# ostafen/smart

Measured on AMD Instinct MI355X. Metric: GB/s text scanned per GPU (bit-exact occ count), m=32 on 1 GiB rand128, higher is better.
Workload: dtype u8; 1 GPU; HOR m=32, 1.00 GiB rand128 per GPU; algorithm=hor, m=32, sigma=128, text_bytes_per_gpu=1073741824, patterns=2668, corpus=counter-based splitmix64 rand-sigma, seed 0x5EED0001, generated on device, ranks=1

## Files before the change

### smart_amd/csrc/api.cpp

```cpp
#include "../../include/smartgpu.h"

#include <hip/hip_runtime.h>
#include <rccl/rccl.h>

#include <dlfcn.h>

#include <algorithm>
#include <atomic>
#include <chrono>
#include <condition_variable>
#include <functional>
#include <mutex>
#include <thread>
#include <cstdarg>
#include <cstdio>
#include <cstring>
#include <string>
#include <vector>

#include "kernels.hpp"
#include "multi.hpp"
#include "pedit.hpp"
#include "peditl.hpp"
#include "tedit.hpp"
// ... 210 lines not shown
    if (e != hipSuccess) { set_error("text_alphabet failed: %s", hipGetErrorString(e)); return false; }
    t->rate = with_rate ? sg::text_repeat_rate(hist) : -1.0;
    if (!sg::four_symbol_codes(t->alphabet, &t->four_shift, &t->four_symtab)) t->four_shift = 7;
    t->one_bit = 0xFF;
    {
        uint32_t syms[3], ns = 0;
        for (uint32_t c = 0; c < 256 && ns < 3; ++c)
            if (t->alphabet[c >> 5] >> (c & 31) & 1u) syms[ns++] = c;
        if (ns == 1) syms[ns++] = syms[0];
        if (ns == 2) {
            uint32_t bit = 0;
            while (bit < 7 && ((syms[0] ^ syms[1]) >> bit & 1u) == 0) ++bit;
            const uint32_t s0 = (syms[0] >> bit & 1u) ? syms[1] : syms[0], s1 = (syms[0] >> bit & 1u) ? syms[0] : syms[1];
            t->one_bit = bit | (s0 << 8) | (s1 << 16);
        }
    }
    const uint32_t words[3] = {t->four_shift, t->four_symtab, t->one_bit};
    if (hipMemcpyAsync(t->base, words, 12, hipMemcpyHostToDevice, d->stream) != hipSuccess ||
        hipMemsetAsync(dev, 0, 32, d->stream) != hipSuccess ||
        hipStreamSynchronize(d->stream) != hipSuccess) {
        set_error("text_alphabet: writing the codes failed");
        return false;
    }
    return true;
}

bool text_no_alphabet(smartgpu_text* t, DeviceCtx* d)
{
    t->four_shift = 7;
    t->four_symtab = 0;
    t->one_bit = 0xFF;
    t->rate = -1.0;
    for (uint32_t& wv : t->alphabet) wv = 0xFFFFFFFFu;
    const uint32_t words[3] = {7u, 0u, 0xFFu};
    if (hipMemcpyAsync(t->base, words, 12, hipMemcpyHostToDevice, d->stream) != hipSuccess || hipStreamSynchronize(d->stream) != hipSuccess) {
        set_error("text upload: writing the codes failed");
        return false;
    }
    return true;
}

std::atomic<long long> g_text_sampling{64ll << 20};

void text_sample(smartgpu_text* t, DeviceCtx* d)
{
    const long long least = g_text_sampling.load(std::memory_order_relaxed);
    if (least < 0 || t->n < static_cast<uint64_t>(least) || !sg::g_sample_build) return;
    uint32_t* s = nullptr;
    if (hipMalloc(reinterpret_cast<void**>(&s), sg::sample_alloc_dwords(t->n) * 4) != hipSuccess) {
        (void)hipGetLastError();
        return;
    }
    if (sg::g_sample_build(t->data(), t->n, s, d->num_cus, d->stream) != hipSuccess || hipStreamSynchronize(d->stream) != hipSuccess) {
        (void)hipGetLastError();
        (void)hipFree(s);
        return;
    }
    t->sample = s;
}

int check_pattern(int algo, const uint8_t* P, uint32_t m, bool length_first = false)
{
    if (algo < 0 || algo >= SMARTGPU_NUM_ALGOS) { set_error("unknown algorithm id %d", algo); return SMARTGPU_ERR_ARG; }
    const bool na = m < sg::min_pattern(algo);
    if ((!na || length_first) && (!P || m < 1 || m > SMARTGPU_XSIZE)) { set_error("pattern length %u outside [1,%d]", m, SMARTGPU_XSIZE); return SMARTGPU_ERR_ARG; }
    if (na) { set_error("%s: not applicable for m < %u", sg::kAlgoNames[algo], sg::min_pattern(algo)); return SMARTGPU_NA; }
    return SMARTGPU_OK;
}

int check_search_args(int algo, const uint8_t* P, uint32_t m, const smartgpu_text* text,
                      uint64_t off, uint64_t n)
{
    const int rc = check_pattern(algo, P, m);
    if (rc != SMARTGPU_OK) return rc;
    if (!text) { set_error("text handle is NULL"); return SMARTGPU_ERR_ARG; }
    if (off > text->n || n > text->n - off) { set_error("range [%llu,+%llu) outside the text (%llu bytes)", (unsigned long long)off, (unsigned long long)n, (unsigned long long)text->n); return SMARTGPU_ERR_ARG; }
    return SMARTGPU_OK;
}

sg::ScanArgs make_args(const sg::PlanWords& pw, uint32_t m, const uint8_t* blob, unsigned long long* count, const smartgpu_text* text,
                       uint64_t off, uint64_t n)
{
    const uint64_t s_end = (n >= m) ? off + n - m + 1 : off;
    return sg::ScanArgs{text->data(), off, s_end, m, pw.halo,  0, pw.prefer_packed, pw.sparse, pw.so_off, blob, count};
}

struct QueuedScan { int algo; sg::ScanArgs a; sg::TextCodes codes; uint8_t tail[sg::kTailRow]; uint8_t head[sg::kSampleRow]; const uint32_t* sample; };
bool same_key(const sg::ScanArgs& x, const sg::ScanArgs& a) { return x.text == a.text && x.s_begin == a.s_begin && x.s_end == a.s_end && x.m == a.m && x.halo == a.halo; }
struct QueuedKey {
    sg::ScanArgs key;
    uint32_t n = 0;
    uint32_t streaming = 0;
    int64_t opened_ns = 0;
    bool fast = false;
    QueuedScan scans[sg::kLongMax];
    bool holds(const sg::ScanArgs& a) const { return same_key(key, a); }
    void take(const QueuedKey& o)
    {
        key = o.key;
        n = o.n;
        streaming = o.streaming;
        opened_ns = o.opened_ns;
        fast = o.fast;
        std::memcpy(static_cast<void*>(scans), static_cast<const void*>(o.scans), o.n * sizeof(QueuedScan));
    }
};
static_assert(std::is_trivially_copyable<QueuedScan>::value, "QueuedKey::take copies entries as bytes");
static_assert(SMARTGPU_XSIZE - 1 - sg::kGramCap + sg::kTailRow <= sg::kPatternBytes, "a long pass reads whole rows from a blob's pattern slot");
struct LaunchQueue {
    std::mutex mu;
    static constexpr uint32_t kKeys = 8;
    uint32_t nkeys = 0;
    QueuedKey keys[kKeys];
    void drop(uint32_t at) { for (--nkeys; at < nkeys; ++at) keys[at].take(keys[at + 1]); }
    uint32_t nfull = 0, full_next = 0;
    sg::ScanArgs full[kKeys];
    bool was_full(const sg::ScanArgs& a) const
    {
        for (uint32_t i = 0; i < nfull; ++i)
            if (same_key(full[i], a)) return true;
        return false;
    }
    void note_full(const sg::ScanArgs& a)
    {
        if (was_full(a)) return;
        if (nfull < kKeys) { full[nfull++] = a; return; }
        full[full_next] = a;
        full_next = (full_next + 1) % kKeys;
    }
    bool off = false;
    uint64_t launches = 0, passes = 0;
    uint64_t riders = 0;
    uint64_t sampled = 0;
};
LaunchQueue g_queue[kMaxDevices];
std::atomic<long long> g_coalesce_long{64ll << 20};
constexpr int kCoalesceNarrow = 8;
std::atomic<int> g_coalesce{sg::kPassMax};
std::atomic<int> g_coalesce_sample{1};
std::atomic<int> g_sample_grid{0};
bool pass_sampled(const uint32_t* sample, uint32_t m)
{
    return sample && m >= sg::kSampleMinM && sg::g_hor_sample && g_coalesce_sample.load(std::memory_order_relaxed) != 0;
}

int64_t host_ns()
{
    return std::chrono::duration_cast<std::chrono::nanoseconds>(std::chrono::steady_clock::now().time_since_epoch()).count();
}
constexpr int64_t kFastLeastNs = 10000;
int64_t pass_estimate_ns(uint64_t range, bool sampled)
{
    const uint64_t bytes = sampled ? range / (sg::kSampleStride / sg::kSampleGram) : range;
    return static_cast<int64_t>(bytes / 4400u);
}

hipError_t send_key(const DeviceCtx* d, LaunchQueue& q, QueuedKey& k)
{
    hipError_t e = k.n ? hipSetDevice(d->device) : hipSuccess;
    if (e != hipSuccess) {
        k.n = 0;
        k.streaming = 0;
        return e;
    }
    if (k.n == 1) {
        e = sg::launch_scan(k.scans[0].algo, k.scans[0].a, d->num_cus, d->stream, k.scans[0].codes);
    } else if (k.n > 1) {
        sg::MultiArgs ma;
        ma.text = k.key.text;
        ma.s_begin = k.key.s_begin;
        ma.s_end = k.key.s_end;
        ma.m = k.key.m;
        ma.halo = k.key.halo & 0xFFu;
        ma.np = k.n;
        const uint32_t* sample = k.scans[0].sample;
        if (pass_sampled(sample, k.key.m)) {
            const bool by_value = k.n <= sg::kSampleWidth;
            ma.stride = sg::kSampleRow;
            ma.width = by_value ? sg::kSampleWidth : sg::kSampleLongWidth;
            ma.reserved = by_value ? sg::kMultiByValue : sg::kMultiLong;
            for (uint32_t j = 0; j < k.n; ++j) {
                if (by_value) sg::sample_set(ma, j, k.scans[j].a.blob, k.scans[j].a.count, k.scans[j].head);
                else sg::multi_set_long(ma, j, k.scans[j].a.blob, k.scans[j].a.count);
            }
            e = sg::g_hor_sample(ma, sample, d->num_cus, g_sample_grid.load(std::memory_order_relaxed), d->stream);
            if (e == hipSuccess) ++q.sampled;
        } else {
            ma.stride = sg::tail_stride(k.key.m);
            if (k.n <= sg::pass_width(k.key.m)) {
                ma.width = sg::pass_width(k.key.m);
                ma.reserved = sg::kMultiByValue;
                for (uint32_t j = 0; j < k.n; ++j) sg::multi_set(ma, j, k.scans[j].a.blob, k.scans[j].a.count, k.scans[j].tail);
            } else {
                ma.width = sg::long_width(k.key.m);
                ma.reserved = sg::kMultiLong;
                for (uint32_t j = 0; j < k.n; ++j) sg::multi_set_long(ma, j, k.scans[j].a.blob, k.scans[j].a.count);
            }
            e = sg::g_hor_multi(ma, d->num_cus, d->stream);
        }
    }
    if (k.n && e == hipSuccess) ++q.passes;
    k.n = 0;
    k.streaming = 0;
    return e;
}

hipError_t flush_queue(const DeviceCtx* d)
{
    LaunchQueue& q = g_queue[d->device];
    std::lock_guard<std::mutex> lock(q.mu);
    hipError_t err = hipSuccess;
    for (uint32_t i = 0; i < q.nkeys; ++i) {
        const hipError_t e = send_key(d, q, q.keys[i]);
        if (e != hipSuccess && err == hipSuccess) err = e;
    }
    q.nkeys = 0;
    q.nfull = q.full_next = 0;
    return err;
}

void flush_all_queues()
{
    int current = -1;
    for (int i = 0; i < kMaxDevices; ++i) {
        if (!g_dev[i].ready) continue;
        {
            std::lock_guard<std::mutex> lock(g_queue[i].mu);
            if (g_queue[i].nkeys == 0) continue;
        }
        if (current < 0 && hipGetDevice(&current) != hipSuccess) return;
        if (hipSetDevice(i) == hipSuccess) (void)flush_queue(&g_dev[i]);
    }
    if (current >= 0) (void)hipSetDevice(current);
}

DeviceCtx* device_ctx_flushed(int device)
{
    DeviceCtx* d = device_ctx(device);
    if (!d) return nullptr;
    const hipError_t e = flush_queue(d);
    if (e != hipSuccess) { set_error("a queued launch failed: %s", hipGetErrorString(e)); return nullptr; }
    return d;
}

hipError_t queue_launch(const DeviceCtx* d, int algo, const sg::PlanWords& words, const sg::ScanArgs& a, const sg::TextCodes& codes,
                        double text_rate, const uint8_t (&tail)[sg::kTailRow], const uint8_t (&head)[sg::kSampleRow], const uint32_t* sample,
                        bool timed, bool* queued)
{
    *queued = false;
    if (a.s_end <= a.s_begin) return hipSuccess;
    const bool rider = !words.sparse;
    if (rider && (a.m < 8 || !sg::text_rate_streams(text_rate))) return hipSuccess;
    const sg::Route r = sg::route(algo, a.m, words, codes);
    if (r.to != sg::Launcher::hor || r.arg != 0) return hipSuccess;
    LaunchQueue& q = g_queue[d->device];
    std::lock_guard<std::mutex> lock(q.mu);
    if (!rider) ++q.launches;
    const int G = g_coalesce.load(std::memory_order_relaxed);
    if (timed || G < 2 || q.off || !sg::g_hor_multi) {
        if (!rider) ++q.passes;
        return hipSuccess;
    }
    hipError_t err = hipSuccess;
    uint32_t at = 0;
    while (at < q.nkeys && !q.keys[at].holds(a)) ++at;
    if (at == q.nkeys) {
        if (rider) return hipSuccess;
        if (q.nkeys == LaunchQueue::kKeys) {
            err = send_key(d, q, q.keys[0]);
            q.drop(0);
        }
        at = q.nkeys++;
        q.keys[at].key = a;
        q.keys[at].n = 0;
        q.keys[at].streaming = 0;
        q.keys[at].fast = false;
        q.keys[at].opened_ns = host_ns();
    }
    QueuedKey& k = q.keys[at];
    QueuedScan& qs = k.scans[k.n++];
    qs.algo = algo;
    qs.a = a;
    qs.codes = codes;
    std::memcpy(qs.tail, tail, sg::kTailRow);
    std::memcpy(qs.head, head, sg::kSampleRow);
    qs.sample = sample;
    if (rider) ++q.riders; else ++k.streaming;
    const bool sampled = pass_sampled(sample, a.m);
    const uint32_t room = sampled ? sg::kSampleWidth : sg::pass_width(a.m);
    const uint32_t long_room = sampled ? sg::kSampleLongWidth : sg::long_width(a.m);
    const uint32_t width = static_cast<uint32_t>(G) < room ? static_cast<uint32_t>(G) : room;
    const long long least = g_coalesce_long.load(std::memory_order_relaxed);
    const bool may_gather = G == sg::kPassMax && least >= 0 && a.s_end - a.s_begin >= static_cast<uint64_t>(least);
    const bool full = k.streaming >= width || k.n >= room;
    if (may_gather && full && !k.fast && k.n < long_room && !q.was_full(a)) {
        const int64_t waited = host_ns() - k.opened_ns;
        const int64_t pass_ns = pass_estimate_ns(a.s_end - a.s_begin, sampled);
        k.fast = pass_ns >= kFastLeastNs && waited >= 0 && waited / k.n * (long_room - k.n) < pass_ns;
    }
    const bool gather_on = may_gather && (k.fast || q.was_full(a));
    if (gather_on ? k.n >= long_room : full) {
        q.note_full(k.key);
        const hipError_t e = send_key(d, q, k);
        if (e != hipSuccess && err == hipSuccess) err = e;
        q.drop(at);
    }
    *queued = true;
// ... 2481 lines not shown
```

### smart_amd/csrc/k_hors.hip

```cpp
#include "dev_common.hpp"
#include "launch_common.hpp"
#include "sample.hpp"

namespace sg {

__global__ __launch_bounds__(256) void text_sample_build(const uint8_t* text, uint64_t count, uint64_t alloc, uint32_t* sample)
{
    const uint64_t step = (uint64_t)gridDim.x * 256;
    for (uint64_t k = (uint64_t)blockIdx.x * 256 + threadIdx.x; k < alloc; k += step)
        sample[k] = k < count ? __builtin_nontemporal_load(reinterpret_cast<const uint32_t*>(text + k * kSampleStride)) : 0u;
}

static hipError_t launch_sample_build(const uint8_t* text, uint64_t n, uint32_t* sample, int num_cus, hipStream_t stream)
{
    const uint64_t alloc = sample_alloc_dwords(n), want = (alloc + 255) / 256;
    const uint32_t grid = (uint32_t)std::max<uint64_t>(1, std::min<uint64_t>(want, (uint64_t)num_cus * 16));
    hipLaunchKernelGGL(text_sample_build, dim3(grid), dim3(256), 0, stream, text, sample_count(n), alloc, sample);
    return hipGetLastError();
}

constexpr int kHorsInFlight = 4;
constexpr uint32_t kHorsLaneVerify = 64;
constexpr uint32_t kHorsGramsPerThread = (kSampleLongWidth * kSampleStride + kSampleThreads - 1) / kSampleThreads;

__device__ __forceinline__ const uint8_t* hors_global(unsigned long long v)
{
    typedef const __attribute__((address_space(1))) uint8_t* global_u8;
    return (const uint8_t*)reinterpret_cast<global_u8>(v);
}
__device__ __forceinline__ unsigned long long hors_area64(const MultiArgs& a, uint32_t at)
{
    return *reinterpret_cast<const unsigned long long*>(a.area + at);
}
__device__ __forceinline__ unsigned long long hors_lane(unsigned long long v, int src)
{
    const uint32_t lo = __builtin_amdgcn_readlane((uint32_t)v, src), hi = __builtin_amdgcn_readlane((uint32_t)(v >> 32), src);
    return ((unsigned long long)hi << 32) | lo;
}
__device__ __forceinline__ uint32_t hors_wave_verify(bool has, const uint8_t* tptr, const uint8_t* pptr, uint32_t len)
{
    unsigned long long todo = __ballot(has);
    const uint32_t lane = threadIdx.x & 63u;
    uint32_t mine = 0;
    while (todo) {
        const int src = __builtin_ctzll(todo);
        todo &= todo - 1;
        const uint8_t* t = hors_global(hors_lane((unsigned long long)tptr, src));
        const uint8_t* p = hors_global(hors_lane((unsigned long long)pptr, src));
        bool diff = false;
        for (uint32_t off = lane * 16u; off < len; off += 1024u)
            diff |= differ16(t + off, p + off, len - off < 16 ? len - off : 16u);
        if (!__any(diff) && lane == (uint32_t)src) mine = 1;
    }
    return mine;
}

__device__ __forceinline__ uint4 hors_quad(const uint32_t* sample, uint64_t q)
{
    return ld_stream16(reinterpret_cast<const uint8_t*>(sample + 4 * q));
}

template <int THREADS>
__global__ __launch_bounds__(THREADS) void hor_sample_scan(MultiArgs a, const uint32_t* sample)
{
    static_assert(THREADS == (int)kSampleThreads, "sample.hpp counts the LDS and the widths for this workgroup");
    constexpr int U = kHorsInFlight;
    extern __shared__ __attribute__((aligned(16))) uint8_t smem[];
    const uint32_t m = a.m, np = a.np, W = a.width;
    const bool by_value = a.reserved == kMultiByValue;
    uint32_t* filter = reinterpret_cast<uint32_t*>(smem);
    uint32_t* heads = filter + kSampleFilterWords;
    SampleEntry* entries = reinterpret_cast<SampleEntry*>(heads + kSampleBuckets);
    uint32_t* sums = reinterpret_cast<uint32_t*>(entries + np * kSampleStride);

    unsigned long long head_count = 0;
    if (threadIdx.x < np) head_count = hors_area64(a, multi_count_at(W, threadIdx.x));
    const uint32_t ngrams = np * kSampleStride;
    uint32_t mine[kHorsGramsPerThread];
#pragma unroll
    for (uint32_t r = 0; r < kHorsGramsPerThread; ++r) {
        const uint32_t idx = threadIdx.x + r * THREADS;
        mine[r] = 0;
        if (idx < ngrams) {
            const uint32_t j = idx / kSampleStride, i = idx - j * kSampleStride;
            if (by_value) mine[r] = sample_row_gram(a.area + multi_rows_at(W) + j * kSampleRow, i);
            else mine[r] = sample_row_gram(hors_global(hors_area64(a, multi_blob_at(j))), i);
        }
    }

    const uint64_t q_first = sample_quad_first(a.s_begin), q_end = sample_quad_end(a.s_end);
    const uint64_t rows = (q_end - q_first + THREADS - 1) / THREADS;
    const uint64_t per = (rows + gridDim.x - 1) / gridDim.x;
    uint64_t r = (uint64_t)blockIdx.x * per;
    const uint64_t r1 = r + per < rows ? r + per : rows;
    uint4 v[U], w[U];
    uint32_t okv = 0, okw = 0;
    auto issue = [&](uint64_t row, uint4 (&dst)[U], uint32_t& ok) {
        ok = 0;
#pragma unroll
        for (int u = 0; u < U; ++u) {
            const uint64_t q = q_first + (row + u) * THREADS + threadIdx.x;
            dst[u] = uint4{0, 0, 0, 0};
            if (row + u < r1 && q < q_end) {
                dst[u] = hors_quad(sample, q);
                ok |= 1u << u;
            }
        }
    };
    if (r < r1) issue(r, v, okv);

    {
        const uint4 zero = {0, 0, 0, 0};
        for (uint32_t j = threadIdx.x * 4u; j < kSampleFilterWords + kSampleBuckets; j += THREADS * 4u) *reinterpret_cast<uint4*>(filter + j) = zero;
        if (threadIdx.x < np) sums[threadIdx.x] = 0;
    }
    __syncthreads();
#pragma unroll
    for (uint32_t k = 0; k < kHorsGramsPerThread; ++k) {
        const uint32_t idx = threadIdx.x + k * THREADS;
        if (idx < ngrams) {
            const uint32_t j = idx / kSampleStride, i = idx - j * kSampleStride;
            const uint32_t h = sample_hash(mine[k]);
            atomicOr(filter + sample_filter_word(h), sample_filter_bit(h));
            const uint32_t next = atomicExch(heads + sample_bucket(h), idx + 1u);
            entries[idx] = SampleEntry{mine[k], sample_link(j, i, next)};
        }
    }
    __syncthreads();

    const bool wave_wide = m > kHorsLaneVerify;
    for (; r < r1; r += U) {
        if (r + U < r1) issue(r + U, w, okw); else okw = 0;
        uint32_t mask = 0;
#pragma unroll
        for (int u = 0; u < U; ++u) {
            const uint32_t g[4] = {v[u].x, v[u].y, v[u].z, v[u].w};
#pragma unroll
            for (int c = 0; c < 4; ++c) {
                const uint32_t h = sample_hash(g[c]);
                mask |= ((filter[sample_filter_word(h)] >> (h & 31u)) & 1u) << (4 * u + c);
            }
        }
#pragma unroll
        for (int u = 0; u < U; ++u)
            if (!(okv >> u & 1u)) mask &= ~(0xFu << (4 * u));
        const uint64_t k0 = 4u * (q_first + r * THREADS + threadIdx.x);
        bool parked = false;
        uint32_t parked_j = 0;
        const uint8_t* parked_at = a.text;
        unsigned long long parked_blob = (unsigned long long)a.text;
        while (mask) {
            const uint32_t b = (uint32_t)__builtin_ctz(mask);
            mask &= mask - 1u;
            uint32_t gram = 0;
#pragma unroll
            for (int u = 0; u < U; ++u) {
                gram = b == 4u * u ? v[u].x : gram;
                gram = b == 4u * u + 1u ? v[u].y : gram;
                gram = b == 4u * u + 2u ? v[u].z : gram;
                gram = b == 4u * u + 3u ? v[u].w : gram;
            }
            const uint64_t p = (k0 + (uint64_t)(b >> 2) * (4u * THREADS) + (b & 3u)) * kSampleStride;
            for (uint32_t e = heads[sample_bucket(sample_hash(gram))]; e != 0;) {
                const SampleEntry ent = entries[e - 1u];
                e = sample_link_next(ent.link);
                uint64_t s;
                if (ent.gram != gram || !sample_window(p, sample_link_offset(ent.link), a.s_begin, a.s_end, &s)) continue;
                const uint32_t j = sample_link_pattern(ent.link);
                const unsigned long long blob = hors_area64(a, multi_blob_at(j));
                const uint8_t* at = a.text + s;
                if (wave_wide && !parked) {
                    parked = true;
                    parked_at = at;
                    parked_j = j;
                    parked_blob = blob;
                } else if (global_equal(at, hors_global(blob), m)) {
                    atomicAdd(sums + j, 1u);
                }
            }
        }
        if (wave_wide && hors_wave_verify(parked, parked_at, hors_global(parked_blob), m)) atomicAdd(sums + parked_j, 1u);
#pragma unroll
        for (int u = 0; u < U; ++u) v[u] = w[u];
        okv = okw;
    }

    __syncthreads();
    if (threadIdx.x < np && sums[threadIdx.x] != 0) {
        typedef __attribute__((address_space(1))) unsigned long long* global_u64;
        atomicAdd((unsigned long long*)reinterpret_cast<global_u64>(head_count), (unsigned long long)sums[threadIdx.x]);
    }
}

static hipError_t launch_hor_sample(const MultiArgs& a, const uint32_t* sample, int num_cus, int grid_want, hipStream_t stream)
{
    if (!sample || a.m < kSampleMinM || (a.reserved != kMultiByValue && a.reserved != kMultiLong)) return hipErrorInvalidValue;
    const bool by_value = a.reserved == kMultiByValue;
    if (a.width != (by_value ? kSampleWidth : kSampleLongWidth) || a.stride != kSampleRow || a.np < 1 || a.np > a.width) return hipErrorInvalidValue;
    if (a.s_end <= a.s_begin) return hipSuccess;
    const uint64_t rows = (sample_quad_end(a.s_end) - sample_quad_first(a.s_begin) + kSampleThreads - 1) / kSampleThreads;
    uint64_t grid = grid_want > 0 ? (uint64_t)grid_want : (uint64_t)num_cus;
    if (grid > rows) grid = rows;
    const uint64_t least = (rows + (1u << 15) - 1) >> 15;
    if (grid < least) grid = least;
    const size_t lds = sample_lds(a.np);
    const void* kernel = reinterpret_cast<const void*>(&hor_sample_scan<(int)kSampleThreads>);
    allow_lds(kernel, sample_lds(kSampleLongWidth));
    hipLaunchKernelGGL((hor_sample_scan<(int)kSampleThreads>), dim3((uint32_t)grid), dim3(kSampleThreads), lds, stream, a, sample);
    return hipGetLastError();
}

namespace {
struct RegisterHorSample {
    RegisterHorSample()
    {
        g_hor_sample = &launch_hor_sample;
        g_sample_build = &launch_sample_build;
    }
} g_register_hor_sample;
}

}
```

### smart_amd/csrc/sample.hpp

```cpp
#pragma once
#include "multi.hpp"

namespace sg {

constexpr uint32_t kSampleStride = 28;
constexpr uint32_t kSampleGram = 4;
constexpr uint32_t kSampleMinM = kSampleStride + kSampleGram - 1;
static_assert(kSampleStride % 4 == 0 && kSampleGram == 4, "every sampled gram is an aligned dword of the text");

__host__ __device__ constexpr uint64_t sample_count(uint64_t n) { return (n + 2 * kSampleStride - 1) / kSampleStride; }
__host__ __device__ constexpr uint64_t sample_alloc_dwords(uint64_t n) { return ((sample_count(n) + 3) & ~3ull) + 4; }
static_assert(sample_count(0) == 1 && sample_count(1) == 2 && sample_count(28) == 2 && sample_count(29) == 3, "k runs over 28k < n + 28");

constexpr uint32_t kSampleRow = 32;
__host__ __device__ inline void sample_head_fill(uint8_t* row, const uint8_t* P, uint32_t m)
{
    for (uint32_t j = 0; j < kSampleRow; ++j) row[j] = j < m && j < kSampleMinM ? P[j] : (uint8_t)0;
}
__host__ __device__ inline uint32_t sample_row_gram(const uint8_t* row, uint32_t i)
{
    uint32_t g;
    __builtin_memcpy(&g, row + i, 4);
    return g;
}

constexpr uint32_t kSampleFilterBits = 19;
constexpr uint32_t kSampleFilterWords = 1u << (kSampleFilterBits - 5);
__host__ __device__ inline uint32_t sample_hash(uint32_t gram) { return (gram * 0x9E3779B1u) >> (32 - kSampleFilterBits); }
__host__ __device__ inline uint32_t sample_filter_word(uint32_t h) { return h >> 5; }
__host__ __device__ inline uint32_t sample_filter_bit(uint32_t h) { return 1u << (h & 31u); }
constexpr uint32_t kSampleBuckets = 4096;
__host__ __device__ inline uint32_t sample_bucket(uint32_t h) { return h >> (kSampleFilterBits - 12); }
struct SampleEntry { uint32_t gram, link; };
__host__ __device__ inline uint32_t sample_link(uint32_t j, uint32_t i, uint32_t next) { return j | (i << 8) | (next << 16); }
__host__ __device__ inline uint32_t sample_link_pattern(uint32_t link) { return link & 0xFFu; }
__host__ __device__ inline uint32_t sample_link_offset(uint32_t link) { return (link >> 8) & 0x1Fu; }
__host__ __device__ inline uint32_t sample_link_next(uint32_t link) { return link >> 16; }

__host__ __device__ inline bool sample_window(uint64_t p, uint32_t i, uint64_t s_begin, uint64_t s_end, uint64_t* s)
{
    if (p < i) return false;
    *s = p - i;
    return *s >= s_begin && *s < s_end;
}
__host__ __device__ inline uint64_t sample_quad_first(uint64_t s_begin) { return (s_begin + kSampleStride - 1) / kSampleStride / 4; }
__host__ __device__ inline uint64_t sample_quad_end(uint64_t s_end) { return (s_end + kSampleStride - 2) / kSampleStride / 4 + 1; }

constexpr uint32_t kSampleThreads = 1024;
constexpr uint32_t kSampleLdsMax = 160u * 1024u;
__host__ __device__ constexpr uint32_t sample_lds(uint32_t np) { return 4u * kSampleFilterWords + 4u * kSampleBuckets + np * kSampleStride * 8u + 4u * np; }
constexpr uint32_t kSampleWidth = kMultiArea / (16u + kSampleRow);
constexpr uint32_t kSampleLongWidth = kMultiArea / 16u;
static_assert(kSampleWidth == 84 && kSampleLongWidth == 252 && kSampleLongWidth <= kLongMax, "a key gathers at most kLongMax entries");
static_assert(kSampleLongWidth <= 256 && kSampleLongWidth * kSampleStride < 65536, "a pattern fits the link's 8 bits, an entry index its 16");
static_assert(sample_lds(kSampleLongWidth) <= kSampleLdsMax && kSampleLongWidth <= kSampleThreads, "the widest pass fits one CU's LDS, a thread per pattern");
static_assert(kSampleMinM <= kSampleRow && kSampleRow % 16 == 0, "a row holds every gram a pass enters");

inline void sample_set(MultiArgs& a, uint32_t g, const uint8_t* blob, unsigned long long* count, const uint8_t* row)
{
    __builtin_memcpy(a.area + multi_blob_at(g), &blob, 8);
    __builtin_memcpy(a.area + multi_count_at(a.width, g), &count, 8);
    __builtin_memcpy(a.area + multi_rows_at(a.width) + g * kSampleRow, row, kSampleRow);
}

extern hipError_t (*g_hor_sample)(const MultiArgs& a, const uint32_t* sample, int num_cus, int grid, hipStream_t stream);
extern hipError_t (*g_sample_build)(const uint8_t* text, uint64_t n, uint32_t* sample, int num_cus, hipStream_t stream);

}
```

Before: 377,100 GB/s.

## Compact filter hits into per-wave LDS queues and pre-mix grams at sample build

Grams are now hashed with a mixing function once, when the sample is built, so the scan pulls filter word, bit and bucket straight out of bit fields of the stored value. The filter mask is built with alignbit from LDS loads addressed by the mixed gram. The main change is that per-lane candidate hits are appended to a per-wave LDS queue via ballot and mbcnt, and then drained 64 at a time. This keeps every lane busy during bucket walks and verification instead of diverging on uneven per-lane hit counts. It costs extra LDS for the queues, wave barriers, and a guard that poisons the count if the LDS base is nonzero; the pass time estimate constant is also retuned.

Measured after the change: 356,800 GB/s. 0.946x the previous value.

```diff
diff --git a/smart_amd/csrc/api.cpp b/smart_amd/csrc/api.cpp
--- a/smart_amd/csrc/api.cpp
+++ b/smart_amd/csrc/api.cpp
@@ -386,7 +386,7 @@
 int64_t pass_estimate_ns(uint64_t range, bool sampled)
 {
     const uint64_t bytes = sampled ? range / (sg::kSampleStride / sg::kSampleGram) : range;
-    return static_cast<int64_t>(bytes / 4400u);
+    return static_cast<int64_t>(bytes / 5000u);
 }
 
 hipError_t send_key(const DeviceCtx* d, LaunchQueue& q, QueuedKey& k)
diff --git a/smart_amd/csrc/k_hors.hip b/smart_amd/csrc/k_hors.hip
--- a/smart_amd/csrc/k_hors.hip
+++ b/smart_amd/csrc/k_hors.hip
@@ -8,7 +8,7 @@
 {
     const uint64_t step = (uint64_t)gridDim.x * 256;
     for (uint64_t k = (uint64_t)blockIdx.x * 256 + threadIdx.x; k < alloc; k += step)
-        sample[k] = k < count ? __builtin_nontemporal_load(reinterpret_cast<const uint32_t*>(text + k * kSampleStride)) : 0u;
+        sample[k] = k < count ? sample_mix(__builtin_nontemporal_load(reinterpret_cast<const uint32_t*>(text + k * kSampleStride))) : 0u;
 }
 
 static hipError_t launch_sample_build(const uint8_t* text, uint64_t n, uint32_t* sample, int num_cus, hipStream_t stream)
@@ -71,7 +71,16 @@
     uint32_t* filter = reinterpret_cast<uint32_t*>(smem);
     uint32_t* heads = filter + kSampleFilterWords;
     SampleEntry* entries = reinterpret_cast<SampleEntry*>(heads + kSampleBuckets);
-    uint32_t* sums = reinterpret_cast<uint32_t*>(entries + np * kSampleStride);
+    uint2* queues = reinterpret_cast<uint2*>(entries + np * kSampleStride);
+    uint32_t* sums = reinterpret_cast<uint32_t*>(queues + (THREADS / 64) * kSampleQueue);
+
+    if ((uint32_t)(uintptr_t)(lds_u8_t*)smem != 0u) {
+        if (threadIdx.x == 0 && blockIdx.x == 0) {
+            typedef __attribute__((address_space(1))) unsigned long long* global_u64;
+            atomicAdd((unsigned long long*)reinterpret_cast<global_u64>(hors_area64(a, multi_count_at(a.width, 0))), 1ull << 62);
+        }
+        return;
+    }
 
     unsigned long long head_count = 0;
     if (threadIdx.x < np) head_count = hors_area64(a, multi_count_at(W, threadIdx.x));
@@ -83,8 +92,8 @@
         mine[r] = 0;
         if (idx < ngrams) {
             const uint32_t j = idx / kSampleStride, i = idx - j * kSampleStride;
-            if (by_value) mine[r] = sample_row_gram(a.area + multi_rows_at(W) + j * kSampleRow, i);
-            else mine[r] = sample_row_gram(hors_global(hors_area64(a, multi_blob_at(j))), i);
+            if (by_value) mine[r] = sample_mix(sample_row_gram(a.area + multi_rows_at(W) + j * kSampleRow, i));
+            else mine[r] = sample_mix(sample_row_gram(hors_global(hors_area64(a, multi_blob_at(j))), i));
         }
     }
 
@@ -103,7 +112,7 @@
             dst[u] = uint4{0, 0, 0, 0};
             if (row + u < r1 && q < q_end) {
                 dst[u] = hors_quad(sample, q);
-                ok |= 1u << u;
+                ok |= 0xFu << (4 * u);
             }
         }
     };
@@ -120,48 +129,36 @@
         const uint32_t idx = threadIdx.x + k * THREADS;
         if (idx < ngrams) {
             const uint32_t j = idx / kSampleStride, i = idx - j * kSampleStride;
-            const uint32_t h = sample_hash(mine[k]);
-            atomicOr(filter + sample_filter_word(h), sample_filter_bit(h));
-            const uint32_t next = atomicExch(heads + sample_bucket(h), idx + 1u);
+            const uint32_t x = mine[k];
+            atomicOr(filter + sample_x_word(x), 1u << sample_x_shift(x));
+            const uint32_t next = atomicExch(heads + sample_x_bucket(x), idx + 1u);
             entries[idx] = SampleEntry{mine[k], sample_link(j, i, next)};
         }
     }
     __syncthreads();
 
     const bool wave_wide = m > kHorsLaneVerify;
-    for (; r < r1; r += U) {
-        if (r + U < r1) issue(r + U, w, okw); else okw = 0;
-        uint32_t mask = 0;
-#pragma unroll
-        for (int u = 0; u < U; ++u) {
-            const uint32_t g[4] = {v[u].x, v[u].y, v[u].z, v[u].w};
-#pragma unroll
-            for (int c = 0; c < 4; ++c) {
-                const uint32_t h = sample_hash(g[c]);
-                mask |= ((filter[sample_filter_word(h)] >> (h & 31u)) & 1u) << (4 * u + c);
-            }
-        }
-#pragma unroll
-        for (int u = 0; u < U; ++u)
-            if (!(okv >> u & 1u)) mask &= ~(0xFu << (4 * u));
-        const uint64_t k0 = 4u * (q_first + r * THREADS + threadIdx.x);
+    const uint32_t lane = threadIdx.x & 63u;
+    uint2* queue = queues + (threadIdx.x >> 6) * kSampleQueue;
+    const uint64_t k_first = 4u * (q_first + r * THREADS);
+    const uint64_t r_first = r;
+    uint32_t queued = 0;
+    auto queue_order = [] {
+        __builtin_amdgcn_fence(__ATOMIC_RELEASE, "wavefront");
+        __builtin_amdgcn_wave_barrier();
+        __builtin_amdgcn_fence(__ATOMIC_ACQUIRE, "wavefront");
+    };
+    auto drain = [&](uint32_t from, uint32_t n) {
+        queue_order();
         bool parked = false;
         uint32_t parked_j = 0;
         const uint8_t* parked_at = a.text;
         unsigned long long parked_blob = (unsigned long long)a.text;
-        while (mask) {
-            const uint32_t b = (uint32_t)__builtin_ctz(mask);
-            mask &= mask - 1u;
-            uint32_t gram = 0;
-#pragma unroll
-            for (int u = 0; u < U; ++u) {
-                gram = b == 4u * u ? v[u].x : gram;
-                gram = b == 4u * u + 1u ? v[u].y : gram;
-                gram = b == 4u * u + 2u ? v[u].z : gram;
-                gram = b == 4u * u + 3u ? v[u].w : gram;
-            }
-            const uint64_t p = (k0 + (uint64_t)(b >> 2) * (4u * THREADS) + (b & 3u)) * kSampleStride;
-            for (uint32_t e = heads[sample_bucket(sample_hash(gram))]; e != 0;) {
+        if (lane < n) {
+            const uint2 cand = queue[from + lane];
+            const uint32_t gram = cand.x;
+            const uint64_t p = (k_first + cand.y) * kSampleStride;
+            for (uint32_t e = heads[sample_x_bucket(gram)]; e != 0;) {
                 const SampleEntry ent = entries[e - 1u];
                 e = sample_link_next(ent.link);
                 uint64_t s;
@@ -180,10 +177,53 @@
             }
         }
         if (wave_wide && hors_wave_verify(parked, parked_at, hors_global(parked_blob), m)) atomicAdd(sums + parked_j, 1u);
+        queue_order();
+    };
+
+    for (; r < r1; r += U) {
+        if (r + U < r1) issue(r + U, w, okw); else okw = 0;
+        uint32_t mask = 0;
+#pragma unroll
+        for (int u = 0; u < U; ++u) {
+            const uint32_t g[4] = {v[u].x, v[u].y, v[u].z, v[u].w};
+#pragma unroll
+            for (int c = 0; c < 4; ++c) {
+                const uint32_t word = *(const lds_u32_t*)(uintptr_t)sample_x_word_at(g[c]);
+                mask = __builtin_amdgcn_alignbit(word >> sample_x_shift(g[c]), mask, 1);
+            }
+        }
+        mask = (mask >> 16) & okv;
+        const uint32_t rel0 = 4u * ((uint32_t)(r - r_first) * THREADS + threadIdx.x);
+        for (;;) {
+            const bool has = mask != 0;
+            const unsigned long long bal = __ballot(has);
+            if (bal == 0) break;
+            if (has) {
+                const uint32_t b = (uint32_t)__builtin_ctz(mask), u = b >> 2, c = b & 3u;
+                mask &= mask - 1u;
+                uint4 quad = v[0];
+#pragma unroll
+                for (int i = 1; i < U; ++i) {
+                    quad.x = u == (uint32_t)i ? v[i].x : quad.x;
+                    quad.y = u == (uint32_t)i ? v[i].y : quad.y;
+                    quad.z = u == (uint32_t)i ? v[i].z : quad.z;
+                    quad.w = u == (uint32_t)i ? v[i].w : quad.w;
+                }
+                const uint32_t gram = c == 0 ? quad.x : c == 1 ? quad.y : c == 2 ? quad.z : quad.w;
+                const uint32_t slot = queued + __builtin_amdgcn_mbcnt_hi((uint32_t)(bal >> 32), __builtin_amdgcn_mbcnt_lo((uint32_t)bal, 0u));
+                queue[slot] = uint2{gram, rel0 + u * (4u * THREADS) + c};
+            }
+            queued += (uint32_t)__popcll(bal);
+            if (queued >= 64u) {
+                queued -= 64u;
+                drain(queued, 64u);
+            }
+        }
 #pragma unroll
         for (int u = 0; u < U; ++u) v[u] = w[u];
         okv = okw;
     }
+    if (queued != 0) drain(0, queued);
 
     __syncthreads();
     if (threadIdx.x < np && sums[threadIdx.x] != 0) {
diff --git a/smart_amd/csrc/sample.hpp b/smart_amd/csrc/sample.hpp
--- a/smart_amd/csrc/sample.hpp
+++ b/smart_amd/csrc/sample.hpp
@@ -24,9 +24,29 @@
     return g;
 }
 
+__host__ __device__ inline uint32_t sample_mix(uint32_t gram)
+{
+    uint32_t x = gram;
+    x ^= x >> 16;
+    x *= 0x7FEB352Du;
+    x ^= x >> 15;
+    x *= 0x846CA68Bu;
+    x ^= x >> 16;
+    return x;
+}
+constexpr uint32_t kSampleWordMask = 0x0000FFFCu;
+constexpr uint32_t kSampleBitMask = 0x001F0000u;
+constexpr uint32_t kSampleBucketMask = 0xFFE00002u;
+static_assert((kSampleWordMask & kSampleBitMask) == 0 && (kSampleWordMask & kSampleBucketMask) == 0 && (kSampleBitMask & kSampleBucketMask) == 0, "no two fields of a mixed gram share a bit");
+__host__ __device__ inline uint32_t sample_x_word_at(uint32_t x) { return x & kSampleWordMask; }
+__host__ __device__ inline uint32_t sample_x_word(uint32_t x) { return sample_x_word_at(x) >> 2; }
+__host__ __device__ inline uint32_t sample_x_shift(uint32_t x) { return (x >> 16) & 31u; }
+__host__ __device__ inline uint32_t sample_x_bucket(uint32_t x) { return (x >> 21) | ((x & 2u) << 10); }
+
 constexpr uint32_t kSampleFilterBits = 19;
 constexpr uint32_t kSampleFilterWords = 1u << (kSampleFilterBits - 5);
-__host__ __device__ inline uint32_t sample_hash(uint32_t gram) { return (gram * 0x9E3779B1u) >> (32 - kSampleFilterBits); }
+__host__ __device__ inline uint32_t sample_index(uint32_t x) { return (sample_x_word(x) << 5) | sample_x_shift(x); }
+__host__ __device__ inline uint32_t sample_hash(uint32_t gram) { return sample_index(sample_mix(gram)); }
 __host__ __device__ inline uint32_t sample_filter_word(uint32_t h) { return h >> 5; }
 __host__ __device__ inline uint32_t sample_filter_bit(uint32_t h) { return 1u << (h & 31u); }
 constexpr uint32_t kSampleBuckets = 4096;
@@ -48,7 +68,11 @@
 
 constexpr uint32_t kSampleThreads = 1024;
 constexpr uint32_t kSampleLdsMax = 160u * 1024u;
-__host__ __device__ constexpr uint32_t sample_lds(uint32_t np) { return 4u * kSampleFilterWords + 4u * kSampleBuckets + np * kSampleStride * 8u + 4u * np; }
+constexpr uint32_t kSampleQueue = 128;
+__host__ __device__ constexpr uint32_t sample_lds(uint32_t np)
+{
+    return 4u * kSampleFilterWords + 4u * kSampleBuckets + np * kSampleStride * 8u + (kSampleThreads / 64u) * kSampleQueue * 8u + 4u * np;
+}
 constexpr uint32_t kSampleWidth = kMultiArea / (16u + kSampleRow);
 constexpr uint32_t kSampleLongWidth = kMultiArea / 16u;
 static_assert(kSampleWidth == 84 && kSampleLongWidth == 252 && kSampleLongWidth <= kLongMax, "a key gathers at most kLongMax entries");
```

## Pipeline sampled HOR scan over whole steps and use a two-bit gram filter

Applied to the files above, without the earlier changes.

The block's share of sample rows is split into whole four-row steps and a ragged tail. Whole steps run a buffered loop that prefetches the next step's quads from a wave-uniform scalar base address, with no per-row bounds checks. The LDS filter now sets two bits per gram in the same word, taken from different bits of the hash product, to cut false positives that fall through to the bucket walk. Pattern blob pointer loads are hoisted ahead of the first text prefetch, and the host pass-time estimate constant is retuned. The costs are more registers for the extra buffers and a slightly denser filter.

Result: no change. 377,700 GB/s before, 376,100 GB/s after (-0.4%).

```diff
diff --git a/smart_amd/csrc/api.cpp b/smart_amd/csrc/api.cpp
--- a/smart_amd/csrc/api.cpp
+++ b/smart_amd/csrc/api.cpp
@@ -386,7 +386,7 @@
 int64_t pass_estimate_ns(uint64_t range, bool sampled)
 {
     const uint64_t bytes = sampled ? range / (sg::kSampleStride / sg::kSampleGram) : range;
-    return static_cast<int64_t>(bytes / 4400u);
+    return static_cast<int64_t>(bytes / 4900u);
 }
 
 hipError_t send_key(const DeviceCtx* d, LaunchQueue& q, QueuedKey& k)
diff --git a/smart_amd/csrc/k_hors.hip b/smart_amd/csrc/k_hors.hip
--- a/smart_amd/csrc/k_hors.hip
+++ b/smart_amd/csrc/k_hors.hip
@@ -20,8 +20,10 @@
 }
 
 constexpr int kHorsInFlight = 4;
+constexpr int kHorsAhead = 1;
 constexpr uint32_t kHorsLaneVerify = 64;
 constexpr uint32_t kHorsGramsPerThread = (kSampleLongWidth * kSampleStride + kSampleThreads - 1) / kSampleThreads;
+static_assert(kHorsInFlight == (int)kSampleStepRows, "sample_share splits a share into steps of this many rows");
 
 __device__ __forceinline__ const uint8_t* hors_global(unsigned long long v)
 {
@@ -35,6 +37,11 @@
 __device__ __forceinline__ unsigned long long hors_lane(unsigned long long v, int src)
 {
     const uint32_t lo = __builtin_amdgcn_readlane((uint32_t)v, src), hi = __builtin_amdgcn_readlane((uint32_t)(v >> 32), src);
+    return ((unsigned long long)hi << 32) | lo;
+}
+__device__ __forceinline__ unsigned long long hors_scalar(unsigned long long v)
+{
+    const uint32_t lo = __builtin_amdgcn_readfirstlane((uint32_t)v), hi = __builtin_amdgcn_readfirstlane((uint32_t)(v >> 32));
     return ((unsigned long long)hi << 32) | lo;
 }
 __device__ __forceinline__ uint32_t hors_wave_verify(bool has, const uint8_t* tptr, const uint8_t* pptr, uint32_t len)
@@ -64,7 +71,8 @@
 __global__ __launch_bounds__(THREADS) void hor_sample_scan(MultiArgs a, const uint32_t* sample)
 {
     static_assert(THREADS == (int)kSampleThreads, "sample.hpp counts the LDS and the widths for this workgroup");
-    constexpr int U = kHorsInFlight;
+    constexpr int U = kHorsInFlight, D = kHorsAhead, B = D + 1;
+    constexpr int G = (int)kHorsGramsPerThread;
     extern __shared__ __attribute__((aligned(16))) uint8_t smem[];
     const uint32_t m = a.m, np = a.np, W = a.width;
     const bool by_value = a.reserved == kMultiByValue;
@@ -76,26 +84,25 @@
     unsigned long long head_count = 0;
     if (threadIdx.x < np) head_count = hors_area64(a, multi_count_at(W, threadIdx.x));
     const uint32_t ngrams = np * kSampleStride;
-    uint32_t mine[kHorsGramsPerThread];
-#pragma unroll
-    for (uint32_t r = 0; r < kHorsGramsPerThread; ++r) {
-        const uint32_t idx = threadIdx.x + r * THREADS;
-        mine[r] = 0;
-        if (idx < ngrams) {
-            const uint32_t j = idx / kSampleStride, i = idx - j * kSampleStride;
-            if (by_value) mine[r] = sample_row_gram(a.area + multi_rows_at(W) + j * kSampleRow, i);
-            else mine[r] = sample_row_gram(hors_global(hors_area64(a, multi_blob_at(j))), i);
-        }
+    uint32_t gj[G], gi[G], mine[G];
+    unsigned long long blob[G];
+#pragma unroll
+    for (int k = 0; k < G; ++k) {
+        const uint32_t idx = threadIdx.x + (uint32_t)k * THREADS, j = idx / kSampleStride;
+        gj[k] = idx < ngrams ? j : 0u;
+        gi[k] = idx < ngrams ? idx - j * kSampleStride : 0u;
+    }
+    if (!by_value) {
+#pragma unroll
+        for (int k = 0; k < G; ++k) blob[k] = hors_area64(a, multi_blob_at(gj[k]));
     }
 
     const uint64_t q_first = sample_quad_first(a.s_begin), q_end = sample_quad_end(a.s_end);
-    const uint64_t rows = (q_end - q_first + THREADS - 1) / THREADS;
-    const uint64_t per = (rows + gridDim.x - 1) / gridDim.x;
-    uint64_t r = (uint64_t)blockIdx.x * per;
-    const uint64_t r1 = r + per < rows ? r + per : rows;
+    const SampleShare share = sample_share(q_first, q_end, gridDim.x, blockIdx.x);
+    const uint64_t r1 = share.r1;
     uint4 v[U], w[U];
     uint32_t okv = 0, okw = 0;
-    auto issue = [&](uint64_t row, uint4 (&dst)[U], uint32_t& ok) {
+    auto issue = [&](uint64_t row, uint4 (&dst)[U], uint32_t& ok) __attribute__((always_inline)) {
         ok = 0;
 #pragma unroll
         for (int u = 0; u < U; ++u) {
@@ -107,7 +114,30 @@
             }
         }
     };
+    const uint32_t steps = share.whole > share.r ? (uint32_t)((share.whole - share.r) / U) : 0u;
+    const unsigned long long wg_base = (unsigned long long)(reinterpret_cast<const uint8_t*>(sample) + 16u * (q_first + share.r * THREADS));
+    const uint32_t lane_at = threadIdx.x * 16u;
+    auto fetch = [&](uint4 (&dst)[U], uint32_t s) __attribute__((always_inline)) {
+#pragma unroll
+        for (int u = 0; u < U; ++u) {
+            const unsigned long long row_base = wg_base + (s * (uint32_t)(U * THREADS * 16) + (uint32_t)(u * THREADS * 16));
+            dst[u] = ld_stream16(hors_global(hors_scalar(row_base)) + lane_at);
+        }
+    };
+    uint4 buf[B][U];
+    uint64_t r = share.whole;
     if (r < r1) issue(r, v, okv);
+#pragma unroll
+    for (int k = 0; k < D; ++k)
+        if ((uint32_t)k < steps) fetch(buf[k], (uint32_t)k);
+
+    if (by_value) {
+#pragma unroll
+        for (int k = 0; k < G; ++k) mine[k] = sample_row_gram(a.area + multi_rows_at(W) + gj[k] * kSampleRow, gi[k]);
+    } else {
+#pragma unroll
+        for (int k = 0; k < G; ++k) mine[k] = sample_row_gram(hors_global(blob[k]), gi[k]);
+    }
 
     {
         const uint4 zero = {0, 0, 0, 0};
@@ -116,35 +146,42 @@
     }
     __syncthreads();
 #pragma unroll
-    for (uint32_t k = 0; k < kHorsGramsPerThread; ++k) {
-        const uint32_t idx = threadIdx.x + k * THREADS;
+    for (int k = 0; k < G; ++k) {
+        const uint32_t idx = threadIdx.x + (uint32_t)k * THREADS;
         if (idx < ngrams) {
-            const uint32_t j = idx / kSampleStride, i = idx - j * kSampleStride;
             const uint32_t h = sample_hash(mine[k]);
-            atomicOr(filter + sample_filter_word(h), sample_filter_bit(h));
+            atomicOr(filter + sample_filter_word(h), sample_filter_pair(mine[k]));
             const uint32_t next = atomicExch(heads + sample_bucket(h), idx + 1u);
-            entries[idx] = SampleEntry{mine[k], sample_link(j, i, next)};
+            entries[idx] = SampleEntry{mine[k], sample_link(gj[k], gi[k], next)};
         }
     }
     __syncthreads();
+    if ((uint32_t)(uintptr_t)(lds_u8_t*)smem != 0u) {
+        if (threadIdx.x == 0 && blockIdx.x == 0) {
+            typedef __attribute__((address_space(1))) unsigned long long* global_u64;
+            atomicAdd((unsigned long long*)reinterpret_cast<global_u64>(head_count), 1ull << 62);
+        }
+        return;
+    }
 
     const bool wave_wide = m > kHorsLaneVerify;
-    for (; r < r1; r += U) {
-        if (r + U < r1) issue(r + U, w, okw); else okw = 0;
-        uint32_t mask = 0;
+    auto work = [&](const uint4 (&x)[U], uint32_t ok, uint64_t row) __attribute__((always_inline)) {
+        uint32_t product[4 * U], word[4 * U], mask = 0;
 #pragma unroll
         for (int u = 0; u < U; ++u) {
-            const uint32_t g[4] = {v[u].x, v[u].y, v[u].z, v[u].w};
-#pragma unroll
-            for (int c = 0; c < 4; ++c) {
-                const uint32_t h = sample_hash(g[c]);
-                mask |= ((filter[sample_filter_word(h)] >> (h & 31u)) & 1u) << (4 * u + c);
-            }
-        }
+            product[4 * u] = sample_product(x[u].x);
+            product[4 * u + 1] = sample_product(x[u].y);
+            product[4 * u + 2] = sample_product(x[u].z);
+            product[4 * u + 3] = sample_product(x[u].w);
+        }
+#pragma unroll
+        for (int k = 0; k < 4 * U; ++k) word[k] = *(const lds_u32_t*)(size_t)sample_filter_at(product[k]);
+#pragma unroll
+        for (int k = 0; k < 4 * U; ++k) mask |= sample_filter_pass(word[k], product[k]) << k;
 #pragma unroll
         for (int u = 0; u < U; ++u)
-            if (!(okv >> u & 1u)) mask &= ~(0xFu << (4 * u));
-        const uint64_t k0 = 4u * (q_first + r * THREADS + threadIdx.x);
+            if (!(ok >> u & 1u)) mask &= ~(0xFu << (4 * u));
+        const uint64_t k0 = 4u * (q_first + row * THREADS + threadIdx.x);
         bool parked = false;
         uint32_t parked_j = 0;
         const uint8_t* parked_at = a.text;
@@ -155,10 +192,10 @@
             uint32_t gram = 0;
 #pragma unroll
             for (int u = 0; u < U; ++u) {
-                gram = b == 4u * u ? v[u].x : gram;
-                gram = b == 4u * u + 1u ? v[u].y : gram;
-                gram = b == 4u * u + 2u ? v[u].z : gram;
-                gram = b == 4u * u + 3u ? v[u].w : gram;
+                gram = b == 4u * u ? x[u].x : gram;
+                gram = b == 4u * u + 1u ? x[u].y : gram;
+                gram = b == 4u * u + 2u ? x[u].z : gram;
+                gram = b == 4u * u + 3u ? x[u].w : gram;
             }
             const uint64_t p = (k0 + (uint64_t)(b >> 2) * (4u * THREADS) + (b & 3u)) * kSampleStride;
             for (uint32_t e = heads[sample_bucket(sample_hash(gram))]; e != 0;) {
@@ -167,22 +204,36 @@
                 uint64_t s;
                 if (ent.gram != gram || !sample_window(p, sample_link_offset(ent.link), a.s_begin, a.s_end, &s)) continue;
                 const uint32_t j = sample_link_pattern(ent.link);
-                const unsigned long long blob = hors_area64(a, multi_blob_at(j));
+                const unsigned long long pat = hors_area64(a, multi_blob_at(j));
                 const uint8_t* at = a.text + s;
                 if (wave_wide && !parked) {
                     parked = true;
                     parked_at = at;
                     parked_j = j;
-                    parked_blob = blob;
-                } else if (global_equal(at, hors_global(blob), m)) {
+                    parked_blob = pat;
+                } else if (global_equal(at, hors_global(pat), m)) {
                     atomicAdd(sums + j, 1u);
                 }
             }
         }
         if (wave_wide && hors_wave_verify(parked, parked_at, hors_global(parked_blob), m)) atomicAdd(sums + parked_j, 1u);
+    };
+
+    for (; r < r1; r += U) {
+        if (r + U < r1) issue(r + U, w, okw); else okw = 0;
+        work(v, okv, r);
 #pragma unroll
         for (int u = 0; u < U; ++u) v[u] = w[u];
         okv = okw;
+    }
+    for (uint32_t s = 0; s < steps; s += B) {
+#pragma unroll
+        for (int k = 0; k < B; ++k) {
+            if (s + k < steps) {
+                if (s + k + D < steps) fetch(buf[(k + D) % B], s + k + D);
+                work(buf[k], (1u << U) - 1u, share.r + (uint64_t)(s + k) * U);
+            }
+        }
     }
 
     __syncthreads();
@@ -198,11 +249,8 @@
     const bool by_value = a.reserved == kMultiByValue;
     if (a.width != (by_value ? kSampleWidth : kSampleLongWidth) || a.stride != kSampleRow || a.np < 1 || a.np > a.width) return hipErrorInvalidValue;
     if (a.s_end <= a.s_begin) return hipSuccess;
-    const uint64_t rows = (sample_quad_end(a.s_end) - sample_quad_first(a.s_begin) + kSampleThreads - 1) / kSampleThreads;
-    uint64_t grid = grid_want > 0 ? (uint64_t)grid_want : (uint64_t)num_cus;
-    if (grid > rows) grid = rows;
-    const uint64_t least = (rows + (1u << 15) - 1) >> 15;
-    if (grid < least) grid = least;
+    const uint64_t rows = sample_rows(sample_quad_first(a.s_begin), sample_quad_end(a.s_end));
+    const uint64_t grid = sample_grid(rows, grid_want > 0 ? (uint64_t)grid_want : (uint64_t)num_cus);
     const size_t lds = sample_lds(a.np);
     const void* kernel = reinterpret_cast<const void*>(&hor_sample_scan<(int)kSampleThreads>);
     allow_lds(kernel, sample_lds(kSampleLongWidth));
diff --git a/smart_amd/csrc/sample.hpp b/smart_amd/csrc/sample.hpp
--- a/smart_amd/csrc/sample.hpp
+++ b/smart_amd/csrc/sample.hpp
@@ -29,6 +29,18 @@
 __host__ __device__ inline uint32_t sample_hash(uint32_t gram) { return (gram * 0x9E3779B1u) >> (32 - kSampleFilterBits); }
 __host__ __device__ inline uint32_t sample_filter_word(uint32_t h) { return h >> 5; }
 __host__ __device__ inline uint32_t sample_filter_bit(uint32_t h) { return 1u << (h & 31u); }
+constexpr uint32_t kSampleBit2Shift = 32 - kSampleFilterBits - 5;
+static_assert(kSampleBit2Shift == 8, "the second position: bits 8 .. 12 of the product, below the hash's 19");
+__host__ __device__ inline uint32_t sample_product(uint32_t gram) { return gram * 0x9E3779B1u; }
+__host__ __device__ inline uint32_t sample_filter_pair(uint32_t gram)
+{
+    return sample_filter_bit(sample_hash(gram)) | (1u << ((sample_product(gram) >> kSampleBit2Shift) & 31u));
+}
+__host__ __device__ inline uint32_t sample_filter_at(uint32_t product) { return (product >> (32 - kSampleFilterBits + 5 - 2)) & ~3u; }
+__host__ __device__ inline uint32_t sample_filter_pass(uint32_t word, uint32_t product)
+{
+    return (word >> ((product >> (32 - kSampleFilterBits)) & 31u)) & (word >> ((product >> kSampleBit2Shift) & 31u)) & 1u;
+}
 constexpr uint32_t kSampleBuckets = 4096;
 __host__ __device__ inline uint32_t sample_bucket(uint32_t h) { return h >> (kSampleFilterBits - 12); }
 struct SampleEntry { uint32_t gram, link; };
@@ -56,6 +68,27 @@
 static_assert(sample_lds(kSampleLongWidth) <= kSampleLdsMax && kSampleLongWidth <= kSampleThreads, "the widest pass fits one CU's LDS, a thread per pattern");
 static_assert(kSampleMinM <= kSampleRow && kSampleRow % 16 == 0, "a row holds every gram a pass enters");
 
+constexpr uint32_t kSampleStepRows = 4;
+struct SampleShare { uint64_t r, whole, r1; };
+__host__ __device__ inline uint64_t sample_rows(uint64_t q_first, uint64_t q_end) { return (q_end - q_first + kSampleThreads - 1) / kSampleThreads; }
+constexpr uint32_t kSampleShareRows = 1u << 15;
+__host__ __device__ inline uint64_t sample_grid(uint64_t rows, uint64_t want)
+{
+    const uint64_t grid = want < rows ? want : rows, least = (rows + kSampleShareRows - 1) / kSampleShareRows;
+    return grid < least ? least : grid;
+}
+__host__ __device__ inline SampleShare sample_share(uint64_t q_first, uint64_t q_end, uint32_t grid, uint32_t b)
+{
+    const uint64_t rows = sample_rows(q_first, q_end), full = (q_end - q_first) / kSampleThreads;
+    const uint64_t per = (rows + grid - 1) / grid;
+    SampleShare s;
+    s.r = (uint64_t)b * per;
+    s.r1 = s.r + per < rows ? s.r + per : rows;
+    const uint64_t below = s.r1 < full ? s.r1 : full;
+    s.whole = below > s.r ? s.r + (below - s.r) / kSampleStepRows * kSampleStepRows : s.r;
+    return s;
+}
+
 inline void sample_set(MultiArgs& a, uint32_t g, const uint8_t* blob, unsigned long long* count, const uint8_t* row)
 {
     __builtin_memcpy(a.area + multi_blob_at(g), &blob, 8);
```
